# noisystreet/aither

Hardware: AMD Instinct MI355X
Metric: Mcell-updates/sec per iteration (residual+LU-SGS), 256^3 block; % HBM roofline (higher is better)
Workload: dtype f64

## Files before the change

### aither_amd/csrc/agx_visc_tile.hpp

```cpp
#pragma once

namespace agx {

constexpr int VT_L = 64, VT_R = 8;
constexpr int VT_OI = VT_L - 2, VT_OJ = VT_R - 2;
enum { VS_S0 = 0, VS_SM = 4, VS_SP = 8, VS_AI0 = 12, VS_AJ0 = 15, VS_AJ1 = 18, VS_AK0 = 21,
       VS_AK1 = 24, VS_VOL = 27, VS_WJ = 28, VS_RHO = 29, VS_MU = 30, VS_AI1 = 31, VS_WI = 34,
       VS_FJ = 35, VS_COUNT = 39 };

#ifndef VT_LDSAREA
#define VT_LDSAREA 1
#endif
#ifndef VT_EDGE_BARRIER
#define VT_EDGE_BARRIER __builtin_amdgcn_sched_barrier(0)
#endif
struct VRef { int var, row, lane; };
using VShared = double (*)[VT_L][VS_COUNT];
__device__ __forceinline__ void vt_ld4(VShared sh, const VRef& r, double* o) {
#pragma unroll
  for (int c = 0; c < 4; ++c) o[c] = sh[r.row][r.lane][r.var + c];
}
__device__ __forceinline__ void vt_ld3(VShared sh, const VRef& r, double* o) {
#pragma unroll
  for (int c = 0; c < 3; ++c) o[c] = sh[r.row][r.lane][r.var + c];
}
__device__ __forceinline__ void vt_acc(double (*grad)[4], const double* val, const double* a,
                                       double sg) {
#pragma unroll
  for (int r = 0; r < 3; ++r) {
    const double w = sg * a[r];
#pragma unroll
    for (int c = 0; c < 4; ++c) grad[r][c] = fma(val[c], w, grad[r][c]);
  }
}
struct VtEdge { VRef c0, c1, a0, a1; };
__device__ __forceinline__ void vt_edge(VShared sh, double (*grad)[4], const double* vsum,
                                        const VtEdge& e, double sg) {
  double c0[4], c1[4], a0[3], a1[3], v[4], a[3];
  vt_ld4(sh, e.c0, c0); vt_ld4(sh, e.c1, c1);
  vt_ld3(sh, e.a0, a0); vt_ld3(sh, e.a1, a1);
#pragma unroll
  for (int c = 0; c < 4; ++c) v[c] = 0.25 * (vsum[c] + c0[c] + c1[c]);
#pragma unroll
  for (int r = 0; r < 3; ++r) a[r] = 0.5 * (a0[r] + a1[r]);
  vt_acc(grad, v, a, sg);
  VT_EDGE_BARRIER;
}
struct VtNoWide {
  __device__ __forceinline__ void operator()(double*, double*, double&, double&) const {}
};
template <bool F4, class Wide>
__device__ __forceinline__ void vt_face(VShared sh, const GasDev& g, const VRef& rL,
                                        const VRef& rU, const VRef& rhoL, const VRef& rhoU,
                                        double rhoU_reg, double muU_reg, bool u_in_reg,
                                        const double* uReg, const double* aF, const double* aFm,
                                        const double* aFp, const VtEdge& t1u, const VtEdge& t1l,
                                        const VtEdge& t2u, const VtEdge& t2l, double volL,
                                        double volU, double wL, double wU, double* f,
                                        const Wide& wide) {
  double grad[3][4];
#pragma unroll
  for (int r = 0; r < 3; ++r)
#pragma unroll
    for (int c = 0; c < 4; ++c) grad[r][c] = 0.0;
  double vL[4], vU[4], vsum[4];
  vt_ld4(sh, rL, vL);
  if (u_in_reg) {
#pragma unroll
    for (int c = 0; c < 4; ++c) vU[c] = uReg[c];
  } else {
    vt_ld4(sh, rU, vU);
  }
#pragma unroll
  for (int c = 0; c < 4; ++c) vsum[c] = vL[c] + vU[c];
  {
    double au[3], al[3];
#pragma unroll
    for (int r = 0; r < 3; ++r) { au[r] = 0.5 * (aF[r] + aFp[r]); al[r] = 0.5 * (aF[r] + aFm[r]); }
    vt_acc(grad, vU, au, 1.0);
    vt_acc(grad, vL, al, -1.0);
  }
  __builtin_amdgcn_sched_barrier(0);
  vt_edge(sh, grad, vsum, t1u, 1.0);
  vt_edge(sh, grad, vsum, t1l, -1.0);
  vt_edge(sh, grad, vsum, t2u, 1.0);
  vt_edge(sh, grad, vsum, t2l, -1.0);
  const double inv_vol = fast_rcp(0.5 * (volL + volU));
#pragma unroll
  for (int r = 0; r < 3; ++r)
#pragma unroll
    for (int c = 0; c < 4; ++c) grad[r][c] *= inv_vol;
  const double rL_ = sh[rhoL.row][rhoL.lane][rhoL.var];
  const double mL_ = sh[rhoL.row][rhoL.lane][rhoL.var + 1];
  const double rU_ = u_in_reg ? rhoU_reg : sh[rhoU.row][rhoU.lane][rhoU.var];
  const double mU_ = u_in_reg ? muU_reg : sh[rhoU.row][rhoU.lane][rhoU.var + 1];
  double vf[3], tf, mu;
  if constexpr (F4) {
    double c0[6], c3[6], w0 = 1.0, w3 = 1.0;
    wide(c0, c3, w0, w3);
    const double w1 = wL, w2 = wU;
    const double r01 = fast_rcp(w0 + w1), r12 = fast_rcp(w1 + w2), r23 = fast_rcp(w2 + w3);
    const double t012 = fast_rcp(w0 + w1 + w2), t123 = fast_rcp(w1 + w2 + w3);
    const double q4 = fast_rcp((w0 + w1) + (w2 + w3));
    const double k3 = w1 * w2, k4 = k3 * (w0 + w1);
    auto c4 = [&](double u0, double u1, double u2, double u3) {
      const double g01 = (u1 - u0) * r01, g12 = (u2 - u1) * r12, g23 = (u3 - u2) * r23;
      const double d3a = (g12 - g01) * t012, d3b = (g23 - g12) * t123;
      return u1 + w1 * g12 - k3 * d3a - k4 * ((d3b - d3a) * q4);
    };
#pragma unroll
    for (int c = 0; c < 3; ++c) vf[c] = c4(c0[c], vL[c], vU[c], c3[c]);
    const double rf = c4(c0[4], rL_, rU_, c3[4]);
    const double pf = c4(c0[4] * c0[3], rL_ * vL[3], rU_ * vU[3], c3[4] * c3[3]);
    tf = pf * fast_rcp(rf);
    mu = g.scaling * c4(c0[5], mL_, mU_, c3[5]);
  } else {
    const double iw = fast_rcp(wL + wU);
    const double cD = wU * iw, cU = wL * iw;
#pragma unroll
    for (int c = 0; c < 3; ++c) vf[c] = cD * vU[c] + cU * vL[c];
    const double rf = cD * rU_ + cU * rL_;
    tf = (cD * rU_ * vU[3] + cU * rL_ * vL[3]) * fast_rcp(rf);
    mu = g.scaling * (cD * mU_ + cU * mL_);
  }
  const double lambda = -(2.0 / 3.0) * mu;
  const double trace = grad[0][0] + grad[1][1] + grad[2][2];
  double tau[3];
#pragma unroll
  for (int r = 0; r < 3; ++r) {
    const double mm = (grad[r][0] + grad[0][r]) * aF[0] + (grad[r][1] + grad[1][r]) * aF[1] +
                      (grad[r][2] + grad[2][r]) * aF[2];
    tau[r] = lambda * trace * aF[r] + mu * mm;
  }
  const double kk = conductivity(g, tf) * g.scaling;
  const double tg = grad[0][3] * aF[0] + grad[1][3] * aF[1] + grad[2][3] * aF[2];
  f[0] = tau[0];
  f[1] = tau[1];
  f[2] = tau[2];
  f[3] = dot3(tau, vf) + kk * tg;
}

template <bool F4>
__global__ void __launch_bounds__(VT_L * VT_R)
k_visc_tile(SlabDev b, GasDev g, SolverDev sp, double cfl, int gx, int gy) {
  __shared__ double sh[VT_R][VT_L][VS_COUNT];
  constexpr int LO = F4 ? 2 : 1;
  constexpr int OI = F4 ? VT_L - 4 : VT_OI;
  const int l = threadIdx.x, ty = threadIdx.y;
  const long S = (long)gx * gy * b.nk;
  const int P = gridDim.x;
  const int rr = P % 8 == 0 ? (int)(blockIdx.x % 8) * (P / 8) + (int)(blockIdx.x / 8)
                            : (int)blockIdx.x;
  long s_pos = S * rr / P;
  const long s_end = S * (rr + 1) / P;
  while (s_pos < s_end) {
  const int col = (int)(s_pos / b.nk);
  const int k0 = (int)(s_pos - (long)col * b.nk);
  const int k1 = (int)min((long)b.nk, k0 + (s_end - s_pos));
  s_pos += k1 - k0;
  const int ci = (col % gx) * OI - LO + l, cj = (col / gx) * VT_OJ - 1 + ty;
  const bool inner = l >= LO && l < LO + OI && ty >= 1 && ty <= VT_OJ;
  const bool own = inner && ci < b.ni && cj < b.nj;
  const bool do_i = l >= LO && l <= LO + OI && ty >= 1 && ty <= VT_OJ && ci <= b.ni && cj < b.nj;
  const bool do_j = ty >= 1 && l >= LO && l < LO + OI && cj <= b.nj && ci < b.ni;
  const int ic = min(ci, F4 ? b.ni + 1 : b.ni), jc = min(cj, F4 ? b.nj + 1 : b.nj);
  const unsigned qc = (unsigned)(b.idx(ic, jc, 0) * 8);
  const unsigned sk = (unsigned)(b.sxy * 8), sj = (unsigned)(b.sx * 8);
  const int kcmax = b.nk + b.ng - 1, kfmax = b.nk + b.ng;
  auto ld_state = [&](int k, double* s4, double& rho, double& mu) {
    const unsigned q = qc + (unsigned)min(k, kcmax) * sk;
    rho = b.ldb(b.st + 0, q);
    s4[0] = b.ldb(b.st + 1, q); s4[1] = b.ldb(b.st + 2, q); s4[2] = b.ldb(b.st + 3, q);
    s4[3] = rho > 0.0 ? b.ldb(b.st + 4, q) * fast_rcp(rho * g.R) : 0.0;
    mu = rho > 0.0 ? viscosity(g, s4[3]) : 0.0;
  };
  auto rq_state = [&](int k, double* raw) {
    const unsigned q = qc + (unsigned)min(k, kcmax) * sk;
#pragma unroll
    for (int e = 0; e < 5; ++e) raw[e] = b.ldb(b.st + e, q);
  };
  auto cv_state = [&](const double* raw, double* s4, double& rho, double& mu) {
    rho = raw[0];
    s4[0] = raw[1]; s4[1] = raw[2]; s4[2] = raw[3];
    s4[3] = rho > 0.0 ? raw[4] * fast_rcp(rho * g.R) : 0.0;
    mu = rho > 0.0 ? viscosity(g, s4[3]) : 0.0;
  };
  auto ld_avec = [&](int d, unsigned q, double* a3) {
    const double mag = b.ldb(PL_FA + 4 * d + 3, q);
    a3[0] = b.ldb(PL_FA + 4 * d + 0, q) * mag; a3[1] = b.ldb(PL_FA + 4 * d + 1, q) * mag;
    a3[2] = b.ldb(PL_FA + 4 * d + 2, q) * mag;
  };
  auto rq_avec = [&](int d, unsigned q, double* raw) {
#pragma unroll
    for (int c = 0; c < 4; ++c) raw[c] = b.ldb(PL_FA + 4 * d + c, q);
  };
  auto cv_avec = [&](const double* raw, double* a3) {
    a3[0] = raw[0] * raw[3]; a3[1] = raw[1] * raw[3]; a3[2] = raw[2] * raw[3];
  };
  auto PUT4 = [&](int var, const double* v) {
#pragma unroll
    for (int c = 0; c < 4; ++c) sh[ty][l][var + c] = v[c];
  };
  auto PUT3 = [&](int var, const double* v) {
#pragma unroll
    for (int c = 0; c < 3; ++c) sh[ty][l][var + c] = v[c];
  };
  auto LD4 = [&](int var, int row, int lane, double* o) {
#pragma unroll
    for (int c = 0; c < 4; ++c) o[c] = sh[row][lane][var + c];
  };
  auto LD3 = [&](int var, int row, int lane, double* o) {
#pragma unroll
    for (int c = 0; c < 3; ++c) o[c] = sh[row][lane][var + c];
  };
  int kk = k0 - 1;
  double R1, MU1, V1, WK0, WK1, AK2[3], AIp[3] = {0, 0, 0}, AJp[3] = {0, 0, 0};
  double S2[4] = {0, 0, 0, 0}, R2 = 0, MU2 = 0, WK2 = 0, RM = 0, MUM = 0, WKM = 0;
  double EJ[7] = {0, 0, 0, 0, 0, 0, 0};
  const bool ej_row = F4 && (ty == 1 || ty == VT_R - 1);
  const unsigned qej = (unsigned)(b.idx(ic, ty == 1 ? jc - 2 : min(jc + 1, b.nj + 1), 0) * 8);
  {
    double t4[4], t3[3], r, m;
    const unsigned qk = qc + (unsigned)kk * sk;
    ld_state(kk, t4, r, m);
    PUT4(VS_S0, t4);
    if (!F4) PUT4(VS_SM, t4);
    sh[ty][l][VS_RHO] = r; sh[ty][l][VS_MU] = m;
    ld_state(kk + 1, t4, R1, MU1);
    PUT4(VS_SP, t4);
    if (F4) {
      ld_state(kk - 1, t4, RM, MUM);
      PUT4(VS_SM, t4);
      ld_state(kk + 2, S2, R2, MU2);
      WKM = b.ldb(PL_WID + 2, qk - sk);
      WK2 = b.ldb(PL_WID + 2, qc + (unsigned)min(kk + 2, kcmax) * sk);
    }
    ld_avec(0, qk, t3); PUT3(VS_AI0, t3);
    ld_avec(0, qk + sk, t3); PUT3(VS_AI1, t3);
    ld_avec(1, qk, t3); PUT3(VS_AJ0, t3);
    ld_avec(1, qk + sk, t3); PUT3(VS_AJ1, t3);
    ld_avec(2, qk, t3); PUT3(VS_AK0, t3);
    ld_avec(2, qk + sk, t3); PUT3(VS_AK1, t3);
    ld_avec(2, qc + (unsigned)min(kk + 2, kfmax) * sk, AK2);
    if (!VT_LDSAREA || l == VT_L - 1) ld_avec(0, qk + 8, AIp);
    if (!VT_LDSAREA || ty == VT_R - 1) ld_avec(1, qk + sj, AJp);
    sh[ty][l][VS_VOL] = b.ldb(PL_VOL, qk); V1 = b.ldb(PL_VOL, qk + sk);
    WK0 = b.ldb(PL_WID + 2, qk); WK1 = b.ldb(PL_WID + 2, qk + sk);
    sh[ty][l][VS_WI] = b.ldb(PL_WID + 0, qk); sh[ty][l][VS_WJ] = b.ldb(PL_WID + 1, qk);
  }
  double fk_lo[4] = {0, 0, 0, 0};
  const int tu = min(ty + 1, VT_R - 1), td = max(ty - 1, 0);
  const int lr = min(l + 1, VT_L - 1), ll = max(l - 1, 0);
  for (; kk < k1; ++kk) {
    const bool pre = kk < k0;
    __syncthreads();
    double fi[4] = {0, 0, 0, 0}, fj[4] = {0, 0, 0, 0}, fk_up[4] = {0, 0, 0, 0};
    const VRef me0{VS_S0, ty, l}, meP{VS_SP, ty, l}, meM{VS_SM, ty, l};
    const VRef meR{VS_RHO, ty, l};
    if (do_i && !pre) {
      double aF[3], aFm[3];
      vt_ld3(sh, VRef{VS_AI0, ty, l}, aF); vt_ld3(sh, VRef{VS_AI0, ty, ll}, aFm);
      if (VT_LDSAREA && l < VT_L - 1) vt_ld3(sh, VRef{VS_AI0, ty, lr}, AIp);
      const VtEdge ju{{VS_S0, tu, l}, {VS_S0, tu, ll}, {VS_AJ0, tu, l}, {VS_AJ0, tu, ll}};
      const VtEdge jl{{VS_S0, td, l}, {VS_S0, td, ll}, {VS_AJ0, ty, l}, {VS_AJ0, ty, ll}};
      const VtEdge ku{meP, {VS_SP, ty, ll}, {VS_AK1, ty, l}, {VS_AK1, ty, ll}};
      const VtEdge kl{meM, {VS_SM, ty, ll}, {VS_AK0, ty, l}, {VS_AK0, ty, ll}};
      auto wide = [&](double* c0, double* c3, double& w0, double& w3) {
        const int l0 = max(l - 2, 0);
        vt_ld4(sh, VRef{VS_S0, ty, l0}, c0); vt_ld4(sh, VRef{VS_S0, ty, lr}, c3);
        c0[4] = sh[ty][l0][VS_RHO]; c0[5] = sh[ty][l0][VS_MU]; w0 = sh[ty][l0][VS_WI];
        c3[4] = sh[ty][lr][VS_RHO]; c3[5] = sh[ty][lr][VS_MU]; w3 = sh[ty][lr][VS_WI];
      };
      vt_face<F4>(sh, g, VRef{VS_S0, ty, ll}, me0, VRef{VS_RHO, ty, ll}, meR, 0.0, 0.0, false,
                  nullptr, aF, aFm, AIp, ju, jl, ku, kl, sh[ty][ll][VS_VOL], sh[ty][l][VS_VOL],
                  sh[ty][ll][VS_WI], sh[ty][l][VS_WI], fi, wide);
    }
    double racc[4];
#pragma unroll
    for (int c = 0; c < 4; ++c) racc[c] = fi[c] - __shfl_down(fi[c], 1, 64);
    __builtin_amdgcn_sched_barrier(0);
    if (do_j && !pre) {
      double aF[3], aFm[3];
      vt_ld3(sh, VRef{VS_AJ0, ty, l}, aF); vt_ld3(sh, VRef{VS_AJ0, td, l}, aFm);
      if (VT_LDSAREA && ty < VT_R - 1) vt_ld3(sh, VRef{VS_AJ0, tu, l}, AJp);
      const VtEdge iu{{VS_S0, ty, lr}, {VS_S0, td, lr}, {VS_AI0, ty, lr}, {VS_AI0, td, lr}};
      const VtEdge il{{VS_S0, ty, ll}, {VS_S0, td, ll}, {VS_AI0, ty, l}, {VS_AI0, td, l}};
      const VtEdge ku{meP, {VS_SP, td, l}, {VS_AK1, ty, l}, {VS_AK1, td, l}};
      const VtEdge kl{meM, {VS_SM, td, l}, {VS_AK0, ty, l}, {VS_AK0, td, l}};
      auto wide = [&](double* c0, double* c3, double& w0, double& w3) {
        if (ty == 1) {
#pragma unroll
          for (int c = 0; c < 6; ++c) c0[c] = EJ[c];
          w0 = EJ[6];
        } else {
          const int t0 = max(ty - 2, 0);
          vt_ld4(sh, VRef{VS_S0, t0, l}, c0);
          c0[4] = sh[t0][l][VS_RHO]; c0[5] = sh[t0][l][VS_MU]; w0 = sh[t0][l][VS_WJ];
        }
        if (ty == VT_R - 1) {
#pragma unroll
          for (int c = 0; c < 6; ++c) c3[c] = EJ[c];
          w3 = EJ[6];
        } else {
          vt_ld4(sh, VRef{VS_S0, tu, l}, c3);
          c3[4] = sh[tu][l][VS_RHO]; c3[5] = sh[tu][l][VS_MU]; w3 = sh[tu][l][VS_WJ];
        }
      };
      vt_face<F4>(sh, g, VRef{VS_S0, td, l}, me0, VRef{VS_RHO, td, l}, meR, 0.0, 0.0, false,
                  nullptr, aF, aFm, AJp, iu, il, ku, kl, sh[td][l][VS_VOL], sh[ty][l][VS_VOL],
                  sh[td][l][VS_WJ], sh[ty][l][VS_WJ], fj, wide);
    }
#pragma unroll
    for (int c = 0; c < 4; ++c) { sh[ty][l][VS_FJ + c] = fj[c]; racc[c] += fj[c]; }
    __builtin_amdgcn_sched_barrier(0);
    const double R0 = sh[ty][l][VS_RHO], MU0 = sh[ty][l][VS_MU], V0 = sh[ty][l][VS_VOL];
    if (own) {
      double aF[3], aFm[3], SPr[4];
      vt_ld3(sh, VRef{VS_AK1, ty, l}, aF); vt_ld3(sh, VRef{VS_AK0, ty, l}, aFm);
      vt_ld4(sh, meP, SPr);
      const VtEdge iu{{VS_SP, ty, lr}, {VS_S0, ty, lr}, {VS_AI1, ty, lr}, {VS_AI0, ty, lr}};
      const VtEdge il{{VS_SP, ty, ll}, {VS_S0, ty, ll}, {VS_AI1, ty, l}, {VS_AI0, ty, l}};
      const VtEdge ju{{VS_SP, tu, l}, {VS_S0, tu, l}, {VS_AJ1, tu, l}, {VS_AJ0, tu, l}};
      const VtEdge jl{{VS_SP, td, l}, {VS_S0, td, l}, {VS_AJ1, ty, l}, {VS_AJ0, ty, l}};
      auto wide = [&](double* c0, double* c3, double& w0, double& w3) {
        vt_ld4(sh, meM, c0);
        c0[4] = RM; c0[5] = MUM; w0 = WKM;
#pragma unroll
        for (int c = 0; c < 4; ++c) c3[c] = S2[c];
        c3[4] = R2; c3[5] = MU2; w3 = WK2;
      };
      vt_face<F4>(sh, g, me0, meP, meR, meR, R1, MU1, true, SPr, aF, aFm, AK2, iu, il, ju, jl, V0,
                  V1, WK0, WK1, fk_up, wide);
    }
    __builtin_amdgcn_sched_barrier(0);
    double nRaw[5], rAI[4], rAJ[4], rAK[4], rAIp[4] = {0, 0, 0, 0}, rAJp[4] = {0, 0, 0, 0};
    const unsigned qn = qc + (unsigned)(kk + 1) * sk;
    const unsigned qn2 = qc + (unsigned)min(kk + 2, kcmax) * sk;
    rq_state(F4 ? kk + 3 : kk + 2, nRaw);
    rq_avec(0, qn2, rAI);
    rq_avec(1, qn2, rAJ);
    rq_avec(2, qc + (unsigned)min(kk + 3, kfmax) * sk, rAK);
    if (!VT_LDSAREA || l == VT_L - 1) rq_avec(0, qn + 8, rAIp);
    if (!VT_LDSAREA || ty == VT_R - 1) rq_avec(1, qn + sj, rAJp);
    const double nV = b.ldb(PL_VOL, qn2);
    const double nWK = b.ldb(PL_WID + 2, F4 ? qc + (unsigned)min(kk + 3, kcmax) * sk : qn2);
    double nEJ[6] = {0, 0, 0, 0, 0, 0}, nEw = 0;
    if (ej_row) {
      const unsigned qe = qej + (unsigned)(kk + 1) * sk;
#pragma unroll
      for (int e = 0; e < 5; ++e) nEJ[e] = b.ldb(b.st + e, qe);
      nEw = b.ldb(PL_WID + 1, qe);
    }
    const double nwi = b.ldb(PL_WID + 0, qn), nwj = b.ldb(PL_WID + 1, qn);
    __syncthreads();
    if (own && !pre) {
      const unsigned q = qc + (unsigned)kk * sk;
      double res[AGX_NEQ];
#pragma unroll
      for (int e = 1; e < AGX_NEQ; ++e) res[e] = b.ldb(PL_RESID + e, q);
#pragma unroll
      for (int c = 0; c < 4; ++c)
        res[1 + c] += ((racc[c] - sh[ty + 1][l][VS_FJ + c]) + fk_lo[c]) - fk_up[c];
      const double ivol = fast_rcp(V0);
      const double vfac = visc_max_term(g, R0) * visc_term(g, MU0);
      double sr = b.ldb(PL_SPECRAD, q);
      double diag = sp.implicit ? b.ldb(PL_A, q) : 0.0;
      double ai0[3], aj0[3], ak0[3], ak1[3];
      LD3(VS_AI0, ty, l, ai0); LD3(VS_AJ0, ty, l, aj0);
      LD3(VS_AK0, ty, l, ak0); LD3(VS_AK1, ty, l, ak1);
      const double fm[3] = {0.5 * (fast_sqrt(dot3(ai0, ai0)) + fast_sqrt(dot3(AIp, AIp))),
                            0.5 * (fast_sqrt(dot3(aj0, aj0)) + fast_sqrt(dot3(AJp, AJp))),
                            0.5 * (fast_sqrt(dot3(ak0, ak0)) + fast_sqrt(dot3(ak1, ak1)))};
#pragma unroll
      for (int d = 0; d < 3; ++d) {
        const double vsr = vfac * fm[d] * fm[d] * ivol;
        sr += vsr * sp.visc_cfl_coeff;
        diag += 2.0 * vsr;
      }
#pragma unroll
      for (int e = 1; e < AGX_NEQ; ++e) b.stb(PL_RESID + e, q, res[e]);
      b.stb(PL_SPECRAD, q, sr);
      if (sp.implicit) b.stb(PL_A, q, diag);
      b.stb(PL_DT, q, sp.dt_fixed > 0.0 ? sp.dt_fixed : cfl * (V0 * fast_rcp(fmax(sr, 0.0))));
    }
    {
      double t3[3], t4[4];
      double nS[4], nR, nMU, nAI[3], nAJ[3], nAK[3], nAIp[3], nAJp[3];
      cv_state(nRaw, nS, nR, nMU);
      cv_avec(rAI, nAI); cv_avec(rAJ, nAJ); cv_avec(rAK, nAK);
      cv_avec(rAIp, nAIp); cv_avec(rAJp, nAJp);
      LD4(VS_S0, ty, l, t4); PUT4(VS_SM, t4);
      LD4(VS_SP, ty, l, t4); PUT4(VS_S0, t4);
      if (F4) {
        PUT4(VS_SP, S2);
        RM = sh[ty][l][VS_RHO]; MUM = sh[ty][l][VS_MU];
        sh[ty][l][VS_RHO] = R1; R1 = R2; R2 = nR;
        sh[ty][l][VS_MU] = MU1; MU1 = MU2; MU2 = nMU;
#pragma unroll
        for (int c = 0; c < 4; ++c) S2[c] = nS[c];
        if (ej_row) {
          const double rho = nEJ[0];
          EJ[0] = nEJ[1]; EJ[1] = nEJ[2]; EJ[2] = nEJ[3];
          EJ[3] = rho > 0.0 ? nEJ[4] * fast_rcp(rho * g.R) : 0.0;
          EJ[4] = rho;
          EJ[5] = rho > 0.0 ? viscosity(g, EJ[3]) : 0.0;
          EJ[6] = nEw;
        }
      } else {
        PUT4(VS_SP, nS);
        sh[ty][l][VS_RHO] = R1; R1 = nR;
        sh[ty][l][VS_MU] = MU1; MU1 = nMU;
      }
      LD3(VS_AI1, ty, l, t3); PUT3(VS_AI0, t3); PUT3(VS_AI1, nAI);
      LD3(VS_AJ1, ty, l, t3); PUT3(VS_AJ0, t3); PUT3(VS_AJ1, nAJ);
      LD3(VS_AK1, ty, l, t3); PUT3(VS_AK0, t3); PUT3(VS_AK1, AK2);
      sh[ty][l][VS_VOL] = V1; V1 = nV;
      sh[ty][l][VS_WI] = nwi; sh[ty][l][VS_WJ] = nwj;
      if (F4) { WKM = WK0; WK0 = WK1; WK1 = WK2; WK2 = nWK; }
      else { WK0 = WK1; WK1 = nWK; }
#pragma unroll
      for (int c = 0; c < 4; ++c) fk_lo[c] = fk_up[c];
#pragma unroll
      for (int c = 0; c < 3; ++c) { AK2[c] = nAK[c]; AIp[c] = nAIp[c]; AJp[c] = nAJp[c]; }
    }
  }
  __syncthreads();
  }
}

}
```

Before: 1465.

## Rotate LDS ring-buffer offsets and carry k-edge terms across iterations

Replaces the per-k LDS shift copies of state and face-area slots with rotating offset indices, so each step writes only the new plane. In the non-F4 path, the lower k-edge gradient contribution of the i and j faces is carried in registers from the previous k step instead of being re-read from LDS. Face-area magnitudes are kept in registers (with a wave shuffle for the i neighbour) so the spectral-radius square roots are no longer recomputed. This lowers LDS traffic and ALU work at the cost of extra registers, runtime-indexed LDS offsets, and a more complex prologue.

```diff
diff --git a/aither_amd/csrc/agx_visc_tile.hpp b/aither_amd/csrc/agx_visc_tile.hpp
--- a/aither_amd/csrc/agx_visc_tile.hpp
+++ b/aither_amd/csrc/agx_visc_tile.hpp
@@ -4,9 +4,8 @@
 
 constexpr int VT_L = 64, VT_R = 8;
 constexpr int VT_OI = VT_L - 2, VT_OJ = VT_R - 2;
-enum { VS_S0 = 0, VS_SM = 4, VS_SP = 8, VS_AI0 = 12, VS_AJ0 = 15, VS_AJ1 = 18, VS_AK0 = 21,
-       VS_AK1 = 24, VS_VOL = 27, VS_WJ = 28, VS_RHO = 29, VS_MU = 30, VS_AI1 = 31, VS_WI = 34,
-       VS_FJ = 35, VS_COUNT = 39 };
+enum { VS_S = 0, VS_AI = 12, VS_AJ = 15, VS_AK = 18, VS_ASTEP = 9, VS_VOL = 30, VS_WJ = 31,
+       VS_RHO = 32, VS_MU = 33, VS_WI = 34, VS_FJ = 35, VS_COUNT = 39 };
 
 #ifndef VT_LDSAREA
 #define VT_LDSAREA 1
@@ -14,6 +13,9 @@
 #ifndef VT_EDGE_BARRIER
 #define VT_EDGE_BARRIER __builtin_amdgcn_sched_barrier(0)
 #endif
+#ifndef VT_KCARRY
+#define VT_KCARRY 1
+#endif
 struct VRef { int var, row, lane; };
 using VShared = double (*)[VT_L][VS_COUNT];
 __device__ __forceinline__ void vt_ld4(VShared sh, const VRef& r, double* o) {
@@ -34,22 +36,27 @@
   }
 }
 struct VtEdge { VRef c0, c1, a0, a1; };
+__device__ __forceinline__ void vt_edge_val(VShared sh, const double* vsum, const VtEdge& e,
+                                            double* v, double* a) {
+  double c0[4], c1[4], a0[3], a1[3];
+  vt_ld4(sh, e.c0, c0); vt_ld4(sh, e.c1, c1);
+  vt_ld3(sh, e.a0, a0); vt_ld3(sh, e.a1, a1);
+#pragma unroll
+  for (int c = 0; c < 4; ++c) v[c] = 0.25 * (vsum[c] + c0[c] + c1[c]);
+#pragma unroll
+  for (int r = 0; r < 3; ++r) a[r] = 0.5 * (a0[r] + a1[r]);
+}
 __device__ __forceinline__ void vt_edge(VShared sh, double (*grad)[4], const double* vsum,
                                         const VtEdge& e, double sg) {
-  double c0[4], c1[4], a0[3], a1[3], v[4], a[3];
-  vt_ld4(sh, e.c0, c0); vt_ld4(sh, e.c1, c1);
-  vt_ld3(sh, e.a0, a0); vt_ld3(sh, e.a1, a1);
-#pragma unroll
-  for (int c = 0; c < 4; ++c) v[c] = 0.25 * (vsum[c] + c0[c] + c1[c]);
-#pragma unroll
-  for (int r = 0; r < 3; ++r) a[r] = 0.5 * (a0[r] + a1[r]);
+  double v[4], a[3];
+  vt_edge_val(sh, vsum, e, v, a);
   vt_acc(grad, v, a, sg);
   VT_EDGE_BARRIER;
 }
 struct VtNoWide {
   __device__ __forceinline__ void operator()(double*, double*, double&, double&) const {}
 };
-template <bool F4, class Wide>
+template <bool F4, bool KC, class Wide>
 __device__ __forceinline__ void vt_face(VShared sh, const GasDev& g, const VRef& rL,
                                         const VRef& rU, const VRef& rhoL, const VRef& rhoU,
                                         double rhoU_reg, double muU_reg, bool u_in_reg,
@@ -57,7 +64,7 @@
                                         const double* aFp, const VtEdge& t1u, const VtEdge& t1l,
                                         const VtEdge& t2u, const VtEdge& t2l, double volL,
                                         double volU, double wL, double wU, double* f,
-                                        const Wide& wide) {
+                                        const Wide& wide, double* kc = nullptr) {
   double grad[3][4];
 #pragma unroll
   for (int r = 0; r < 3; ++r)
@@ -83,8 +90,15 @@
   __builtin_amdgcn_sched_barrier(0);
   vt_edge(sh, grad, vsum, t1u, 1.0);
   vt_edge(sh, grad, vsum, t1l, -1.0);
-  vt_edge(sh, grad, vsum, t2u, 1.0);
-  vt_edge(sh, grad, vsum, t2l, -1.0);
+  if constexpr (KC) {
+    vt_acc(grad, kc, kc + 4, -1.0);
+    vt_edge_val(sh, vsum, t2u, kc, kc + 4);
+    vt_acc(grad, kc, kc + 4, 1.0);
+    VT_EDGE_BARRIER;
+  } else {
+    vt_edge(sh, grad, vsum, t2u, 1.0);
+    vt_edge(sh, grad, vsum, t2l, -1.0);
+  }
   const double inv_vol = fast_rcp(0.5 * (volL + volU));
 #pragma unroll
   for (int r = 0; r < 3; ++r)
@@ -153,6 +167,8 @@
                             : (int)blockIdx.x;
   long s_pos = S * rr / P;
   const long s_end = S * (rr + 1) / P;
+  int oM = 4, o0 = 0, oP = 8, oA0 = 0, oA1 = VS_ASTEP;
+  constexpr bool KC = VT_KCARRY && !F4;
   while (s_pos < s_end) {
   const int col = (int)(s_pos / b.nk);
   const int k0 = (int)(s_pos - (long)col * b.nk);
@@ -189,6 +205,7 @@
     const double mag = b.ldb(PL_FA + 4 * d + 3, q);
     a3[0] = b.ldb(PL_FA + 4 * d + 0, q) * mag; a3[1] = b.ldb(PL_FA + 4 * d + 1, q) * mag;
     a3[2] = b.ldb(PL_FA + 4 * d + 2, q) * mag;
+    return mag;
   };
   auto rq_avec = [&](int d, unsigned q, double* raw) {
 #pragma unroll
@@ -205,16 +222,10 @@
 #pragma unroll
     for (int c = 0; c < 3; ++c) sh[ty][l][var + c] = v[c];
   };
-  auto LD4 = [&](int var, int row, int lane, double* o) {
-#pragma unroll
-    for (int c = 0; c < 4; ++c) o[c] = sh[row][lane][var + c];
-  };
-  auto LD3 = [&](int var, int row, int lane, double* o) {
-#pragma unroll
-    for (int c = 0; c < 3; ++c) o[c] = sh[row][lane][var + c];
-  };
   int kk = k0 - 1;
   double R1, MU1, V1, WK0, WK1, AK2[3], AIp[3] = {0, 0, 0}, AJp[3] = {0, 0, 0};
+  double MI0, MI1, MJ0, MJ1, MK0, MK1, MK2, MIp = 0;
+  double kci[7] = {0, 0, 0, 0, 0, 0, 0}, kcj[7] = {0, 0, 0, 0, 0, 0, 0};
   double S2[4] = {0, 0, 0, 0}, R2 = 0, MU2 = 0, WK2 = 0, RM = 0, MUM = 0, WKM = 0;
   double EJ[7] = {0, 0, 0, 0, 0, 0, 0};
   const bool ej_row = F4 && (ty == 1 || ty == VT_R - 1);
@@ -223,26 +234,26 @@
     double t4[4], t3[3], r, m;
     const unsigned qk = qc + (unsigned)kk * sk;
     ld_state(kk, t4, r, m);
-    PUT4(VS_S0, t4);
-    if (!F4) PUT4(VS_SM, t4);
+    PUT4(VS_S + o0, t4);
+    if (!F4) PUT4(VS_S + oM, t4);
     sh[ty][l][VS_RHO] = r; sh[ty][l][VS_MU] = m;
     ld_state(kk + 1, t4, R1, MU1);
-    PUT4(VS_SP, t4);
+    PUT4(VS_S + oP, t4);
     if (F4) {
       ld_state(kk - 1, t4, RM, MUM);
-      PUT4(VS_SM, t4);
+      PUT4(VS_S + oM, t4);
       ld_state(kk + 2, S2, R2, MU2);
       WKM = b.ldb(PL_WID + 2, qk - sk);
       WK2 = b.ldb(PL_WID + 2, qc + (unsigned)min(kk + 2, kcmax) * sk);
     }
-    ld_avec(0, qk, t3); PUT3(VS_AI0, t3);
-    ld_avec(0, qk + sk, t3); PUT3(VS_AI1, t3);
-    ld_avec(1, qk, t3); PUT3(VS_AJ0, t3);
-    ld_avec(1, qk + sk, t3); PUT3(VS_AJ1, t3);
-    ld_avec(2, qk, t3); PUT3(VS_AK0, t3);
-    ld_avec(2, qk + sk, t3); PUT3(VS_AK1, t3);
-    ld_avec(2, qc + (unsigned)min(kk + 2, kfmax) * sk, AK2);
-    if (!VT_LDSAREA || l == VT_L - 1) ld_avec(0, qk + 8, AIp);
+    MI0 = ld_avec(0, qk, t3); PUT3(VS_AI + oA0, t3);
+    MI1 = ld_avec(0, qk + sk, t3); PUT3(VS_AI + oA1, t3);
+    MJ0 = ld_avec(1, qk, t3); PUT3(VS_AJ + oA0, t3);
+    MJ1 = ld_avec(1, qk + sk, t3); PUT3(VS_AJ + oA1, t3);
+    MK0 = ld_avec(2, qk, t3); PUT3(VS_AK + oA0, t3);
+    MK1 = ld_avec(2, qk + sk, t3); PUT3(VS_AK + oA1, t3);
+    MK2 = ld_avec(2, qc + (unsigned)min(kk + 2, kfmax) * sk, AK2);
+    if (!VT_LDSAREA || l == VT_L - 1) MIp = ld_avec(0, qk + 8, AIp);
     if (!VT_LDSAREA || ty == VT_R - 1) ld_avec(1, qk + sj, AJp);
     sh[ty][l][VS_VOL] = b.ldb(PL_VOL, qk); V1 = b.ldb(PL_VOL, qk + sk);
     WK0 = b.ldb(PL_WID + 2, qk); WK1 = b.ldb(PL_WID + 2, qk + sk);
@@ -255,8 +266,29 @@
     const bool pre = kk < k0;
     __syncthreads();
     double fi[4] = {0, 0, 0, 0}, fj[4] = {0, 0, 0, 0}, fk_up[4] = {0, 0, 0, 0};
+    const int VS_S0 = VS_S + o0, VS_SP = VS_S + oP, VS_SM = VS_S + oM;
+    const int VS_AI0 = VS_AI + oA0, VS_AI1 = VS_AI + oA1, VS_AJ0 = VS_AJ + oA0;
+    const int VS_AJ1 = VS_AJ + oA1, VS_AK0 = VS_AK + oA0, VS_AK1 = VS_AK + oA1;
     const VRef me0{VS_S0, ty, l}, meP{VS_SP, ty, l}, meM{VS_SM, ty, l};
     const VRef meR{VS_RHO, ty, l};
+    if (KC && pre) {
+      double vL[4], vU[4], vsum[4];
+      vt_ld4(sh, me0, vU);
+      if (do_i) {
+        vt_ld4(sh, VRef{VS_S0, ty, ll}, vL);
+#pragma unroll
+        for (int c = 0; c < 4; ++c) vsum[c] = vL[c] + vU[c];
+        vt_edge_val(sh, vsum, VtEdge{meP, {VS_SP, ty, ll}, {VS_AK1, ty, l}, {VS_AK1, ty, ll}},
+                    kci, kci + 4);
+      }
+      if (do_j) {
+        vt_ld4(sh, VRef{VS_S0, td, l}, vL);
+#pragma unroll
+        for (int c = 0; c < 4; ++c) vsum[c] = vL[c] + vU[c];
+        vt_edge_val(sh, vsum, VtEdge{meP, {VS_SP, td, l}, {VS_AK1, ty, l}, {VS_AK1, td, l}},
+                    kcj, kcj + 4);
+      }
+    }
     if (do_i && !pre) {
       double aF[3], aFm[3];
       vt_ld3(sh, VRef{VS_AI0, ty, l}, aF); vt_ld3(sh, VRef{VS_AI0, ty, ll}, aFm);
@@ -271,9 +303,9 @@
         c0[4] = sh[ty][l0][VS_RHO]; c0[5] = sh[ty][l0][VS_MU]; w0 = sh[ty][l0][VS_WI];
         c3[4] = sh[ty][lr][VS_RHO]; c3[5] = sh[ty][lr][VS_MU]; w3 = sh[ty][lr][VS_WI];
       };
-      vt_face<F4>(sh, g, VRef{VS_S0, ty, ll}, me0, VRef{VS_RHO, ty, ll}, meR, 0.0, 0.0, false,
-                  nullptr, aF, aFm, AIp, ju, jl, ku, kl, sh[ty][ll][VS_VOL], sh[ty][l][VS_VOL],
-                  sh[ty][ll][VS_WI], sh[ty][l][VS_WI], fi, wide);
+      vt_face<F4, KC>(sh, g, VRef{VS_S0, ty, ll}, me0, VRef{VS_RHO, ty, ll}, meR, 0.0, 0.0,
+                      false, nullptr, aF, aFm, AIp, ju, jl, ku, kl, sh[ty][ll][VS_VOL],
+                      sh[ty][l][VS_VOL], sh[ty][ll][VS_WI], sh[ty][l][VS_WI], fi, wide, kci);
     }
     double racc[4];
 #pragma unroll
@@ -306,9 +338,9 @@
           c3[4] = sh[tu][l][VS_RHO]; c3[5] = sh[tu][l][VS_MU]; w3 = sh[tu][l][VS_WJ];
         }
       };
-      vt_face<F4>(sh, g, VRef{VS_S0, td, l}, me0, VRef{VS_RHO, td, l}, meR, 0.0, 0.0, false,
-                  nullptr, aF, aFm, AJp, iu, il, ku, kl, sh[td][l][VS_VOL], sh[ty][l][VS_VOL],
-                  sh[td][l][VS_WJ], sh[ty][l][VS_WJ], fj, wide);
+      vt_face<F4, KC>(sh, g, VRef{VS_S0, td, l}, me0, VRef{VS_RHO, td, l}, meR, 0.0, 0.0,
+                      false, nullptr, aF, aFm, AJp, iu, il, ku, kl, sh[td][l][VS_VOL],
+                      sh[ty][l][VS_VOL], sh[td][l][VS_WJ], sh[ty][l][VS_WJ], fj, wide, kcj);
     }
 #pragma unroll
     for (int c = 0; c < 4; ++c) { sh[ty][l][VS_FJ + c] = fj[c]; racc[c] += fj[c]; }
@@ -329,8 +361,8 @@
         for (int c = 0; c < 4; ++c) c3[c] = S2[c];
         c3[4] = R2; c3[5] = MU2; w3 = WK2;
       };
-      vt_face<F4>(sh, g, me0, meP, meR, meR, R1, MU1, true, SPr, aF, aFm, AK2, iu, il, ju, jl, V0,
-                  V1, WK0, WK1, fk_up, wide);
+      vt_face<F4, false>(sh, g, me0, meP, meR, meR, R1, MU1, true, SPr, aF, aFm, AK2, iu, il, ju,
+                         jl, V0, V1, WK0, WK1, fk_up, wide);
     }
     __builtin_amdgcn_sched_barrier(0);
     double nRaw[5], rAI[4], rAJ[4], rAK[4], rAIp[4] = {0, 0, 0, 0}, rAJp[4] = {0, 0, 0, 0};
@@ -353,6 +385,7 @@
     }
     const double nwi = b.ldb(PL_WID + 0, qn), nwj = b.ldb(PL_WID + 1, qn);
     __syncthreads();
+    const double mi_nb = F4 ? 0.0 : __shfl_down(MI0, 1, 64);
     if (own && !pre) {
       const unsigned q = qc + (unsigned)kk * sk;
       double res[AGX_NEQ];
@@ -365,12 +398,19 @@
       const double vfac = visc_max_term(g, R0) * visc_term(g, MU0);
       double sr = b.ldb(PL_SPECRAD, q);
       double diag = sp.implicit ? b.ldb(PL_A, q) : 0.0;
-      double ai0[3], aj0[3], ak0[3], ak1[3];
-      LD3(VS_AI0, ty, l, ai0); LD3(VS_AJ0, ty, l, aj0);
-      LD3(VS_AK0, ty, l, ak0); LD3(VS_AK1, ty, l, ak1);
-      const double fm[3] = {0.5 * (fast_sqrt(dot3(ai0, ai0)) + fast_sqrt(dot3(AIp, AIp))),
-                            0.5 * (fast_sqrt(dot3(aj0, aj0)) + fast_sqrt(dot3(AJp, AJp))),
-                            0.5 * (fast_sqrt(dot3(ak0, ak0)) + fast_sqrt(dot3(ak1, ak1)))};
+      double fm[3];
+      if constexpr (F4) {
+        double ai0[3], aj0[3], ak0[3], ak1[3];
+        vt_ld3(sh, VRef{VS_AI0, ty, l}, ai0); vt_ld3(sh, VRef{VS_AJ0, ty, l}, aj0);
+        vt_ld3(sh, VRef{VS_AK0, ty, l}, ak0); vt_ld3(sh, VRef{VS_AK1, ty, l}, ak1);
+        fm[0] = 0.5 * (fast_sqrt(dot3(ai0, ai0)) + fast_sqrt(dot3(AIp, AIp)));
+        fm[1] = 0.5 * (fast_sqrt(dot3(aj0, aj0)) + fast_sqrt(dot3(AJp, AJp)));
+        fm[2] = 0.5 * (fast_sqrt(dot3(ak0, ak0)) + fast_sqrt(dot3(ak1, ak1)));
+      } else {
+        fm[0] = 0.5 * (MI0 + (!VT_LDSAREA || l == VT_L - 1 ? MIp : mi_nb));
+        fm[1] = 0.5 * (MJ0 + fast_sqrt(dot3(AJp, AJp)));
+        fm[2] = 0.5 * (MK0 + MK1);
+      }
 #pragma unroll
       for (int d = 0; d < 3; ++d) {
         const double vsr = vfac * fm[d] * fm[d] * ivol;
@@ -384,15 +424,12 @@
       b.stb(PL_DT, q, sp.dt_fixed > 0.0 ? sp.dt_fixed : cfl * (V0 * fast_rcp(fmax(sr, 0.0))));
     }
     {
-      double t3[3], t4[4];
       double nS[4], nR, nMU, nAI[3], nAJ[3], nAK[3], nAIp[3], nAJp[3];
       cv_state(nRaw, nS, nR, nMU);
       cv_avec(rAI, nAI); cv_avec(rAJ, nAJ); cv_avec(rAK, nAK);
       cv_avec(rAIp, nAIp); cv_avec(rAJp, nAJp);
-      LD4(VS_S0, ty, l, t4); PUT4(VS_SM, t4);
-      LD4(VS_SP, ty, l, t4); PUT4(VS_S0, t4);
       if (F4) {
-        PUT4(VS_SP, S2);
+        PUT4(VS_SM, S2);
         RM = sh[ty][l][VS_RHO]; MUM = sh[ty][l][VS_MU];
         sh[ty][l][VS_RHO] = R1; R1 = R2; R2 = nR;
         sh[ty][l][VS_MU] = MU1; MU1 = MU2; MU2 = nMU;
@@ -407,13 +444,15 @@
           EJ[6] = nEw;
         }
       } else {
-        PUT4(VS_SP, nS);
+        PUT4(VS_SM, nS);
         sh[ty][l][VS_RHO] = R1; R1 = nR;
         sh[ty][l][VS_MU] = MU1; MU1 = nMU;
       }
-      LD3(VS_AI1, ty, l, t3); PUT3(VS_AI0, t3); PUT3(VS_AI1, nAI);
-      LD3(VS_AJ1, ty, l, t3); PUT3(VS_AJ0, t3); PUT3(VS_AJ1, nAJ);
-      LD3(VS_AK1, ty, l, t3); PUT3(VS_AK0, t3); PUT3(VS_AK1, AK2);
+      PUT3(VS_AI0, nAI); PUT3(VS_AJ0, nAJ); PUT3(VS_AK0, AK2);
+      { const int t = oM; oM = o0; o0 = oP; oP = t; }
+      { const int t = oA0; oA0 = oA1; oA1 = t; }
+      MI0 = MI1; MI1 = rAI[3]; MJ0 = MJ1; MJ1 = rAJ[3];
+      MK0 = MK1; MK1 = MK2; MK2 = rAK[3]; MIp = rAIp[3];
       sh[ty][l][VS_VOL] = V1; V1 = nV;
       sh[ty][l][VS_WI] = nwi; sh[ty][l][VS_WJ] = nwj;
       if (F4) { WKM = WK0; WK0 = WK1; WK1 = WK2; WK2 = nWK; }
```

Result: no change. 1464 (-0.1%).
